# LukasHaas/PIGEON

Hardware: AMD Instinct MI355X
Metric: images/sec end-to-end (ViT+head+refine), 4x336x336 (higher is better)
Workload: dtype f16

## Files before the change

### include/pigeon_hip.h

```cpp
#ifndef PIGEON_HIP_H
#define PIGEON_HIP_H

#include <stddef.h>
#include <stdint.h>

#ifdef __cplusplus
extern "C" {
#endif

#define PG_OK            0
#define PG_EINVAL       -1
#define PG_ENOMEM       -2
#define PG_EHIP         -3
#define PG_ESTATE       -4

#define PG_DTYPE_F32     0
#define PG_DTYPE_BF16    1
#define PG_DTYPE_F16     2
#define PG_DTYPE_F64     3

#define PG_ABI_VERSION   7

const char* pg_last_error(void);
int pg_abi_version(void);
// ... 143 lines not shown
int pg_comm_rccl_version(void);

int pg_proto_build(const float* train_emb, int panels, int64_t num_train, const int64_t* member_off,
                   const int64_t* member_idx, int64_t num_protos, float* proto_emb, void* stream);
int pg_haversine_matrix(const void* x, int x_dtype, const double* y, int N, int M, double* out, void* stream);
int pg_haversine_pairs(const double* x, const void* y, int y_dtype, int64_t N, double* out, void* stream);
int pg_smooth_labels(const double* distances, int N, int M, double constant, double* out, void* stream);

int pg_haversine_blocks(const double* pts, const int64_t* cell_off, const int64_t* mat_off, int C, double zero_as, double* out,
                        void* stream);
int pg_optics_graph(const double* dist, const int64_t* cell_off, const int64_t* mat_off, int C, int min_samples, int64_t* ordering,
                    double* core, double* reach, int64_t* pred, void* stream);
int pg_optics_plan(int64_t n, int min_samples, int32_t out[4]);
int pg_tune_optics_lds_points(int max_points);

int pg_op_gemm16(int dtype, const void* A, int64_t lda, const void* W, const float* bias, void* out, int64_t ldc,
                 int M, int N, int K, int epi, float qscale, int qcols, const float* aux,
                 int variant, void* stream);
int pg_op_gemm16_ld(int dtype, const void* A, int64_t lda, const void* W, int64_t ldw, const float* bias, void* out,
                    int64_t ldc, int M, int N, int K, int epi, float qscale, int qcols, const float* aux,
                    int variant, void* stream);
int pg_op_rowstat_cast(const float* x, void* x16, int dtype, float* rowstat, int64_t rows, float eps, void* stream);
int pg_op_gemm16_resid_stat(int dtype, const void* A, int64_t lda, const void* W, int64_t ldw, const float* bias, float* X,
                            int64_t ldc, void* x16, int64_t ldx, float* statpart, int M, int N, int K, int variant, void* stream);
int pg_op_rowstat_finalize(const float* statpart, int slots, float* rowstat, int64_t rows, float eps, void* stream);
int pg_op_gemm16_ln(int dtype, const void* A, int64_t lda, const void* W, int64_t ldw, const float* bias, const float* colsum,
                    const float* rowstat, void* out, int64_t ldc, int M, int N, int K, int epi, float qscale, int qcols,
                    int variant, void* stream);
int pg_op_layernorm(const float* x, const float* gamma, const float* beta, void* y, int out_dtype,
                    int64_t rows, float eps, void* stream);
int pg_op_attention(int dtype, const void* qkv, void* out, int n_images, void* stream);
int pg_op_im2col(const void* pixels, int pix_dtype, void* out, int out_dtype, int n_images, void* stream);
int pg_op_token_mean(const float* x, float* out, int n_images, void* stream);
int pg_op_cast_f32(const float* x, void* y, int out_dtype, int64_t n, void* stream);
int pg_op_preln(float* x, const float* cls, const float* pos0, const float* gamma, const float* beta, int64_t rows, float eps,
                void* x16, int x16_dtype, float* rowstat, void* stream);
int pg_op_gemm16_parts(int dtype, const void* A, int64_t lda, const void* W, int64_t ldw, const float* bias, float* parts,
                       int M, int N, int Kp, int S, void* stream);
int pg_op_x3_split(const float* x, void* y3, int64_t rows, int cols, int gelu, void* stream);
int pg_op_x3_layernorm(const float* x, const float* gamma, const float* beta, void* y3, int64_t rows, float eps, void* stream);
int pg_op_attention_f32(const float* qkv, float* out, int n_images, void* stream);
int pg_op_attention_x3(const float* qkv, void* out3, int n_images, void* stream);
int pg_op_x3_im2col(const void* pixels, int pix_dtype, void* out3, int n_images, void* stream);
int pg_op_sum_parts(const float* parts, int S, int64_t part_elems, float* dst, int64_t n, int resid, void* stream);

#ifdef __cplusplus
}
#endif
#endif
```

### pigeon_amd/_lib.py

```python
from __future__ import annotations

import ctypes as C
import os

_HERE = os.path.dirname(os.path.abspath(__file__))
LIB_PATH = os.environ.get("PIGEON_HIP_LIB") or os.path.join(_HERE, "libpigeon_hip.so")

PG_DTYPE_F32, PG_DTYPE_BF16, PG_DTYPE_F16, PG_DTYPE_F64 = 0, 1, 2, 3
EPI_QKV, EPI_GELU, EPI_RESID, EPI_PATCH, EPI_F32, EPI_RESID_STAT, EPI_QKV_LN, EPI_GELU_LN, EPI_GELU_X3 = 0, 1, 2, 3, 4, 5, 6, 7, 8
PROF_CLASSES = ["gemm_qkv", "gemm_out", "gemm_fc1", "gemm_fc2", "gemm_patch", "attention", "layernorm",
                "im2col", "token_mean"]


class PigeonHipError(RuntimeError):
    pass


class VitCfg(C.Structure):
    _fields_ = [("layers", C.c_int32), ("image_size", C.c_int32), ("patch", C.c_int32), ("hidden", C.c_int32),
                ("heads", C.c_int32), ("mlp", C.c_int32), ("ln_eps", C.c_float), ("max_chunk", C.c_int32),
                ("mma_dtype", C.c_int32), ("precise", C.c_int32)]


class Bank(C.Structure):
# ... 64 lines not shown
    "pg_prep_ragged_destroy": (_I, [_P]),
    "pg_prep_ragged_forward": (_I, [_P, _P, _SZ, C.POINTER(PrepItem), _I, _P, _I, _P, _SZ, _P]),
    "pg_proto_build": (_I, [_P, _I, _I64, _P, _P, _I64, _P, _P]),
    "pg_haversine_matrix": (_I, [_P, _I, _P, _I, _I, _P, _P]),
    "pg_haversine_pairs": (_I, [_P, _P, _I, _I64, _P, _P]),
    "pg_smooth_labels": (_I, [_P, _I, _I, _D, _P, _P]),
    "pg_haversine_blocks": (_I, [_P, _P, _P, _I, _D, _P, _P]),
    "pg_optics_graph": (_I, [_P, _P, _P, _I, _I, _P, _P, _P, _P, _P]),
    "pg_optics_plan": (_I, [_I64, _I, C.POINTER(C.c_int32)]),
    "pg_tune_optics_lds_points": (_I, [_I]),
    "pg_head_forward": (_I, [_P, _I, _I, _P, _P, _P, _I, _I, _P, _P, _P, _P, _P, _P]),
    "pg_head_margin": (_I, [_P, _I, _I, _P, _I, _P, _P, _P, _P, _P]),
    "pg_head_certainty": (_I, [_P, _I, _I, _P, _I, _P, _P, _I, _P, _P, _P, _P, _P, _P, _P]),
    "pg_aux_heads_forward": (_I, [_P, _I, _I, _P, _P, _I, _I, _I, _P, _P, _P, _P, _P, _P, _P]),
    "pg_refine_forward": (_I, [C.POINTER(Bank), _P, _I, _I, _P, _P, _P, _I, _I, _F, _D, _P, _P, _P, _P, _P]),
    "pg_refine_forward_ex": (_I, [C.POINTER(Bank), _P, _I, _I, _P, _P, _P, _I, _I, _I, _F, _D, _P, _P, _P, _P, _P, _P]),
    "pg_refine_certainty": (_I, [C.POINTER(Bank), _P, _I, _I, _P, _P, _I, _I, _I, _P, _P, _I, _P, _P, _F, _P, _P, _P, _P, _P]),
    "pg_requeue_append": (_I, [_P, _P, _P, _I, _F, _I, _I64, _I64, _I64, _P, _P, _P, _P, _P, _P]),
    "pg_rows_to_slots": (_I, [_P, _I64, _P, _I, _P, _P]),
    "pg_requeue_take": (_I, [_P, _I64, _I64, _I, _I, _P, _P]),
    "pg_scatter_rows": (_I, [_P, _I64, _P, _I, _P, _I64, _I64, _I64, _I64, _P]),
    "pg_head_wstats": (_I, [_P, _I, _P, _P, _P]),
    "pg_embedding_debias": (_I, [_P, _I64, _I, _P, _P]),
    "pg_op_gemm16": (_I, [_I, _P, _I64, _P, _P, _P, _I64, _I, _I, _I, _I, _F, _I, _P, _I, _P]),
    "pg_op_gemm16_ld": (_I, [_I, _P, _I64, _P, _I64, _P, _P, _I64, _I, _I, _I, _I, _F, _I, _P, _I, _P]),
    "pg_op_rowstat_cast": (_I, [_P, _P, _I, _P, _I64, _F, _P]),
    "pg_op_gemm16_resid_stat": (_I, [_I, _P, _I64, _P, _I64, _P, _P, _I64, _P, _I64, _P, _I, _I, _I, _I, _P]),
    "pg_op_rowstat_finalize": (_I, [_P, _I, _P, _I64, _F, _P]),
    "pg_op_gemm16_ln": (_I, [_I, _P, _I64, _P, _I64, _P, _P, _P, _P, _I64, _I, _I, _I, _I, _F, _I, _I, _P]),
    "pg_op_layernorm": (_I, [_P, _P, _P, _P, _I, _I64, _F, _P]),
    "pg_op_attention": (_I, [_I, _P, _P, _I, _P]),
    "pg_op_im2col": (_I, [_P, _I, _P, _I, _I, _P]),
    "pg_op_token_mean": (_I, [_P, _P, _I, _P]),
    "pg_op_cast_f32": (_I, [_P, _P, _I, _I64, _P]),
    "pg_op_gemm16_parts": (_I, [_I, _P, _I64, _P, _I64, _P, _P, _I, _I, _I, _I, _P]),
    "pg_op_x3_split": (_I, [_P, _P, _I64, _I, _I, _P]),
    "pg_op_x3_layernorm": (_I, [_P, _P, _P, _P, _I64, _F, _P]),
    "pg_op_attention_f32": (_I, [_P, _P, _I, _P]),
    "pg_op_attention_x3": (_I, [_P, _P, _I, _P]),
    "pg_op_x3_im2col": (_I, [_P, _I, _P, _I, _P]),
    "pg_op_sum_parts": (_I, [_P, _I, _I64, _P, _I64, _I, _P]),
    "pg_op_preln": (_I, [_P, _P, _P, _P, _P, _I64, _F, _P, _I, _P, _P]),
    "pg_vit_precise_plan": (_I, [_I, C.POINTER(C.c_int32)]),
}

_lib = None


def load():
    global _lib
    if _lib is not None:
        return _lib
    if not os.path.exists(LIB_PATH):
        raise PigeonHipError(
            f"{LIB_PATH} not found: build it with `python -m pigeon_amd.build` (hipcc, gfx950). "
            "pigeon_amd has no CPU/PyTorch fallback for its hot path.")
    import torch
    lib = C.CDLL(LIB_PATH)
    for name, (res, args) in SIGNATURES.items():
        fn = getattr(lib, name)
        fn.restype = res
        fn.argtypes = args
    _lib = lib
    return lib


# ... 14 lines not shown
```

### pigeon_amd/build.py

```python
from __future__ import annotations

import os
import subprocess
import sys
from concurrent.futures import ThreadPoolExecutor

HERE = os.path.dirname(os.path.abspath(__file__))
CSRC = os.path.join(HERE, "csrc")
OBJ = os.path.join(CSRC, "build")
LIB = os.path.join(HERE, "libpigeon_hip.so")
SOURCES = ["vit.hip", "gemm_plan.hip", "gemm_bf16.hip", "gemm_pp.hip", "gemm_pp6.hip", "gemm_tail.hip", "gemm_mid.hip", "attention.hip", "rowops.hip", "precise.hip",
           "preprocess.hip", "geo_proto.hip", "head.hip", "refine.hip", "certainty.hip", "aux_heads.hip", "requeue.hip", "fingerprint.hip", "comm.hip", "optics.hip"]
HEADERS = [os.path.join(CSRC, "common.h"), os.path.join(CSRC, "pigeon_internal.h"), os.path.join(CSRC, "gemm_epi.h"),
           os.path.join(CSRC, "attention_common.h"), os.path.join(CSRC, "certainty_common.h"),
           os.path.join(os.path.dirname(HERE), "include", "pigeon_hip.h")]
FLAGS = ["--offload-arch=gfx950", "-O3", "-std=c++17", "-fPIC", "-Wall", "-Wno-unused-function"]


def hipcc() -> str:
    for c in (os.environ.get("HIPCC"), "/opt/rocm/bin/hipcc", "hipcc"):
        if c and (os.path.isabs(c) and os.path.exists(c) or not os.path.isabs(c)):
            return c
    return "hipcc"


def _stale(target: str, deps) -> bool:
    if not os.path.exists(target):
        return True
    t = os.path.getmtime(target)
    return any(os.path.getmtime(d) > t for d in deps)


def build(force: bool = False, verbose: bool = True, dev: bool = False) -> str:
    global OBJ, LIB
    obj_dir = os.path.join(CSRC, "build_dev" if dev else "build")
    lib = os.path.join(HERE, "libpigeon_hip_dev.so" if dev else "libpigeon_hip.so")
    flags = FLAGS + (["-DPIGEON_PROBES"] if dev else [])
    return _build(obj_dir, lib, flags, force, verbose, SOURCES)


def _build(OBJ: str, LIB: str, FLAGS, force: bool, verbose: bool, SOURCES) -> str:
    os.makedirs(OBJ, exist_ok=True)
    cc = hipcc()
    jobs = []
# ... 43 lines not shown
```

### pigeon_amd/csrc/pigeon_internal.h

```cpp
#pragma once
#include <hip/hip_runtime.h>
#include <stdint.h>
#include "../../include/pigeon_hip.h"

enum { EPI_QKV = 0, EPI_GELU = 1, EPI_RESID = 2, EPI_PATCH = 3, EPI_F32 = 4, EPI_RESID_STAT = 5, EPI_QKV_LN = 6, EPI_GELU_LN = 7,
       EPI_GELU_X3 = 8 };

struct PgGemmExtra {
    const float* colsum = nullptr;
    const float* rowstat = nullptr;
    void* x16 = nullptr;
    int64_t ldx = 0;
    float* statpart = nullptr;
    int64_t stat_rows = 0;
    int parts = 1;
    int64_t a_part = 0, w_part = 0, c_part = 0;
};

void pg_set_error(const char* fmt, ...) __attribute__((format(printf, 1, 2)));
int pg_check_launch(const char* what);
int pg_default_gemm_variant();
int pg_gemm_grid_cus();
int pg_gemm_raster_gn();
unsigned long long pg_tune_epoch();
int pg_gemm_precise_route(int M, int N, int Ktot, bool resid, const int* cand, int ncand);

enum { PG_GEMM_V_ONE_TILE = 8, PG_GEMM_V_PP = 36, PG_GEMM_V_PP6 = 56, PG_GEMM_V_TAIL = 70, PG_GEMM_V_MID = 71 };
enum PgGemmKernel { PG_GK_NONE = -1, PG_GK_PP6 = 0, PG_GK_PP = 1, PG_GK_MID = 2, PG_GK_TAIL = 3, PG_GK_ONE_TILE = 4 };

#define PG_HIP(call)                                                                          \
    do {                                                                                      \
        hipError_t e__ = (call);                                                              \
        if (e__ != hipSuccess) {                                                              \
            pg_set_error("%s failed: %s (%s:%d)", #call, hipGetErrorString(e__), __FILE__, __LINE__); \
            return PG_EHIP;                                                                   \
        }                                                                                     \
    } while (0)

struct PgFpBuf { const void* data; size_t bytes; uint64_t seed; };
int pg_fingerprint_many(const PgFpBuf* bufs, int n, uint64_t* out, hipStream_t stream);
void pg_fingerprint_host(const void* data, size_t bytes, uint64_t seed, uint64_t out[2]);

int pg_gemm_launch(int dtype, const void* A, int64_t lda, const void* W, int64_t ldw, const float* bias, void* out, int64_t ldc,
                   int M, int N, int K, int epi, float qscale, int qcols, const float* aux, int variant,
                   hipStream_t s, const PgGemmExtra* extra = nullptr);
int pg_layernorm_launch(const float* x, const float* gamma, const float* beta, void* y, int out_dtype,
                        int64_t rows, float eps, hipStream_t s);
int pg_preln_launch(float* x, const float* cls, const float* pos0, const float* gamma, const float* beta,
                    int64_t rows, float eps, hipStream_t s, void* x16 = nullptr, int x16_dtype = 0, float* rowstat = nullptr);
int pg_im2col_launch(const void* pixels, int pix_dtype, void* out, int out_dtype, int n_images, hipStream_t s);
int pg_token_mean_launch(const float* x, float* out, int n_images, hipStream_t s);
int pg_cast_f32_launch(const float* x, void* y, int out_dtype, int64_t n, hipStream_t s);
int pg_rowstat_cast_launch(const float* x, void* x16, int out_dtype, float* rowstat, int64_t rows, float eps, hipStream_t s);
int pg_rowstat_finalize_launch(const float* statpart, int slots, float* rowstat, int64_t rows, float eps, hipStream_t s,
                               unsigned long long* alarm = nullptr, float alarm_sumsq = 0.f);
int pg_count_sat16_launch(const void* buf, int64_t rows, int cols, int64_t ld, int dtype, unsigned long long* counter, hipStream_t s);
int pg_attention_launch(int dtype, const void* qkv, void* out, int n_images, hipStream_t s);
int pg_x3_ln_launch(const float* x, const float* gamma, const float* beta, void* y3, int64_t rows, float eps, hipStream_t s);
int pg_x3_split_launch(const float* x, void* y3, int64_t rows, int C, int gelu, hipStream_t s);
int pg_x3_im2col_launch(const void* pixels, int pix_dtype, void* out3, int n_images, hipStream_t s);
int pg_attention_f32_launch(const float* qkv, float* out, int n_images, hipStream_t s);
bool pg_attention_x3out_available();
int pg_attention_x3out_launch(const float* qkv, void* out3, int n_images, hipStream_t s);
int pg_sum_parts_launch(const float* parts, int S, int64_t part_elems, float* dst, int64_t n, int resid, hipStream_t s);
```

### pigeon_amd/csrc/rowops.hip

```cpp
#include "common.h"
#include "pigeon_internal.h"

template <int OUT>
__global__ __launch_bounds__(256) void layernorm_kernel(const float* __restrict__ x, const float* __restrict__ gamma,
                                                        const float* __restrict__ beta, void* __restrict__ y,
                                                        int64_t rows, float eps) {
    const int lane = threadIdx.x & 63;
    const int64_t row = (int64_t)blockIdx.x * 4 + (threadIdx.x >> 6);
    if (row >= rows) return;
    const float* xr = x + row * VIT_HIDDEN;
    f32x4 v[4];
#pragma unroll
    for (int i = 0; i < 4; ++i) v[i] = *(const f32x4*)(xr + i * 256 + lane * 4);
    float s = 0.f;
#pragma unroll
    for (int i = 0; i < 4; ++i) s += (v[i][0] + v[i][1]) + (v[i][2] + v[i][3]);
    const float mean = wave_sum(s) * (1.0f / VIT_HIDDEN);
    float q = 0.f;
#pragma unroll
    for (int i = 0; i < 4; ++i)
#pragma unroll
        for (int e = 0; e < 4; ++e) { const float d = v[i][e] - mean; q += d * d; }
    const float var = wave_sum(q) * (1.0f / VIT_HIDDEN);
    const float rstd = 1.0f / sqrtf(var + eps);
// ... 200 lines not shown
    } else { pg_set_error("im2col: unsupported pixel dtype %d", pix_dtype); return PG_EINVAL; }
    return pg_check_launch("im2col");
}

__global__ __launch_bounds__(256) void token_mean_kernel(const float* __restrict__ x, float* __restrict__ out) {
    const int img = blockIdx.x >> 2, col = (blockIdx.x & 3) * 256 + threadIdx.x;
    const float* p = x + (int64_t)img * VIT_TOKENS * VIT_HIDDEN + col;
    float s0 = 0.f, s1 = 0.f, s2 = 0.f, s3 = 0.f;
    int t = 0;
    for (; t + 16 <= VIT_TOKENS; t += 16) {
        float v[16];
#pragma unroll
        for (int i = 0; i < 16; ++i) v[i] = p[(int64_t)(t + i) * VIT_HIDDEN];
#pragma unroll
        for (int i = 0; i < 16; i += 4) { s0 += v[i]; s1 += v[i + 1]; s2 += v[i + 2]; s3 += v[i + 3]; }
    }
    for (; t + 4 <= VIT_TOKENS; t += 4) {
        s0 += p[(int64_t)(t + 0) * VIT_HIDDEN];
        s1 += p[(int64_t)(t + 1) * VIT_HIDDEN];
        s2 += p[(int64_t)(t + 2) * VIT_HIDDEN];
        s3 += p[(int64_t)(t + 3) * VIT_HIDDEN];
    }
    for (; t < VIT_TOKENS; ++t) s0 += p[(int64_t)t * VIT_HIDDEN];
    out[(int64_t)img * VIT_HIDDEN + col] = ((s0 + s1) + (s2 + s3)) / (float)VIT_TOKENS;
}

int pg_token_mean_launch(const float* x, float* out, int n_images, hipStream_t s) {
    if (n_images <= 0) return PG_OK;
    hipLaunchKernelGGL(token_mean_kernel, dim3(n_images * 4), dim3(256), 0, s, x, out);
    return pg_check_launch("token_mean");
}

template <typename T>
__global__ __launch_bounds__(256) void f32_to_16_kernel(const float* __restrict__ x, uint16_t* __restrict__ y, int64_t n) {
    int64_t i = ((int64_t)blockIdx.x * 256 + threadIdx.x) * 4;
    const int64_t stride = (int64_t)gridDim.x * 256 * 4;
    for (; i + 3 < n; i += stride) {
        const f32x4 v = *(const f32x4*)(x + i);
        u32x2 pk;
        pk[0] = pack16x2<T>(v[0], v[1]);
        pk[1] = pack16x2<T>(v[2], v[3]);
        *(u32x2*)(y + i) = pk;
    }
    if (i < n) for (int64_t j = i; j < n; ++j) y[j] = T::bits(x[j]);
}

int pg_cast_f32_launch(const float* x, void* y, int out_dtype, int64_t n, hipStream_t s) {
    if (n <= 0) return PG_OK;
    int64_t blocks = (n / 4 + 255) / 256;
    if (blocks > 4096) blocks = 4096;
    if (blocks < 1) blocks = 1;
    if (out_dtype == PG_DTYPE_F16) hipLaunchKernelGGL(f32_to_16_kernel<T_F16>, dim3((unsigned)blocks), dim3(256), 0, s, x, (uint16_t*)y, n);
    else if (out_dtype == PG_DTYPE_BF16) hipLaunchKernelGGL(f32_to_16_kernel<T_BF16>, dim3((unsigned)blocks), dim3(256), 0, s, x, (uint16_t*)y, n);
    else { pg_set_error("cast: bad output dtype %d", out_dtype); return PG_EINVAL; }
    return pg_check_launch("cast_f32");
}

__global__ __launch_bounds__(256) void count_sat16_kernel(const uint16_t* __restrict__ buf, int64_t rows, int cols, int64_t ld,
                                                          int is_f16, unsigned long long* __restrict__ counter) {
    const int64_t vec_per_row = cols / 8;
    const int64_t total = rows * vec_per_row;
    unsigned long long n = 0;
    for (int64_t i = (int64_t)blockIdx.x * 256 + threadIdx.x; i < total; i += (int64_t)gridDim.x * 256) {
        const int64_t r = i / vec_per_row, c = (i - r * vec_per_row) * 8;
        const u32x4 v = *(const u32x4*)(buf + r * ld + c);
#pragma unroll
// ... 19 lines not shown
```

### pigeon_amd/csrc/vit.hip

```cpp
#include "common.h"
#include "pigeon_internal.h"

#include <cmath>
#include <cstdarg>
#include <cstdio>
#include <cstdlib>
#include <cstring>
#include <map>
#include <string>
#include <vector>

static thread_local char g_err[512] = "";

void pg_set_error(const char* fmt, ...) {
    va_list ap;
    va_start(ap, fmt);
    vsnprintf(g_err, sizeof(g_err), fmt, ap);
    va_end(ap);
}
int pg_check_launch(const char* what) {
    hipError_t e = hipGetLastError();
    if (e != hipSuccess) { pg_set_error("launch of %s failed: %s", what, hipGetErrorString(e)); return PG_EHIP; }
    return PG_OK;
}
// ... 344 lines not shown
      RC(pg_gemm_launch(dt, big, VIT_PATCH_KPAD, h->wpatch, VIT_PATCH_KPAD, nullptr, X, VIT_HIDDEN, n * VIT_PATCHES, VIT_HIDDEN, VIT_PATCH_KPAD,
                        EPI_PATCH, 1.f, 0, h->pos, 0, s)); }
    if (!h->ln_fold) { ProfScope p(h, s, 6); RC(pg_preln_launch(X, h->cls, h->pos, h->preg, h->preb, M, eps, s)); }
    if (h->ln_fold) {
        uint16_t* Xn2 = (uint16_t*)((char*)big + align_up((size_t)M * VIT_MLP * 2, 256));
        float* statpart = (float*)((char*)Xn2 + align_up((size_t)M * VIT_HIDDEN * 2, 256));
        float* rsA = (float*)((char*)statpart + align_up((size_t)M * (VIT_HIDDEN / 64) * 8, 256));
        float* rsB = (float*)((char*)rsA + align_up((size_t)M * 8, 256));
        const int slots = VIT_HIDDEN / 64;
        { ProfScope p(h, s, 6); RC(pg_preln_launch(X, h->cls, h->pos, h->preg, h->preb, M, eps, s, Xn, dt, rsA)); }
        SAT(Xn, M, VIT_HIDDEN, VIT_HIDDEN);
        for (int l = 0; l < h->cfg.layers; ++l) {
            const LayerW& L = h->layers[l];
            const bool last = l + 1 == h->cfg.layers;
            PgGemmExtra ex;
            { ProfScope p(h, s, 0);
              ex = PgGemmExtra(); ex.colsum = L.sqkv; ex.rowstat = rsA;
              RC(pg_gemm_launch(dt, Xn, VIT_HIDDEN, L.wqkv, VIT_HIDDEN, L.bqkv, big, 3 * VIT_HIDDEN, (int)M, 3 * VIT_HIDDEN, VIT_HIDDEN,
                                EPI_QKV_LN, kQScale, VIT_HIDDEN, nullptr, 0, s, &ex)); }
            SAT(big, M, 3 * VIT_HIDDEN, 3 * VIT_HIDDEN);
            { ProfScope p(h, s, 5); RC(pg_attention_launch(dt, big, Xn, n, s)); }
            SAT(Xn, M, VIT_HIDDEN, VIT_HIDDEN);
            { ProfScope p(h, s, 1);
              ex = PgGemmExtra(); ex.x16 = Xn2; ex.ldx = VIT_HIDDEN; ex.statpart = statpart;
              RC(pg_gemm_launch(dt, Xn, VIT_HIDDEN, L.wo, VIT_HIDDEN, L.bo, X, VIT_HIDDEN, (int)M, VIT_HIDDEN, VIT_HIDDEN, EPI_RESID_STAT,
                                1.f, 0, nullptr, 0, s, &ex)); }
            SAT(Xn2, M, VIT_HIDDEN, VIT_HIDDEN);
            { ProfScope p(h, s, 6); RC(pg_rowstat_finalize_launch(statpart, slots, rsB, M, eps, s, h->range_alarm, h->range_alarm_sumsq)); }
            { ProfScope p(h, s, 2);
              ex = PgGemmExtra(); ex.colsum = L.s1; ex.rowstat = rsB;
              RC(pg_gemm_launch(dt, Xn2, VIT_HIDDEN, L.w1, VIT_HIDDEN, L.b1, big, VIT_MLP, (int)M, VIT_MLP, VIT_HIDDEN, EPI_GELU_LN, 1.f, 0,
                                nullptr, 0, s, &ex)); }
            SAT(big, M, VIT_MLP, VIT_MLP);
            { ProfScope p(h, s, 3);
              if (last) {
                  RC(pg_gemm_launch(dt, big, VIT_MLP, L.w2, VIT_MLP, L.b2, X, VIT_HIDDEN, (int)M, VIT_HIDDEN, VIT_MLP, EPI_RESID, 1.f, 0, nullptr, 0, s));
              } else {
                  ex = PgGemmExtra(); ex.x16 = Xn; ex.ldx = VIT_HIDDEN; ex.statpart = statpart;
                  RC(pg_gemm_launch(dt, big, VIT_MLP, L.w2, VIT_MLP, L.b2, X, VIT_HIDDEN, (int)M, VIT_HIDDEN, VIT_MLP, EPI_RESID_STAT, 1.f, 0,
                                    nullptr, 0, s, &ex));
              } }
            if (!last) SAT(Xn, M, VIT_HIDDEN, VIT_HIDDEN);
            if (!last) { ProfScope p(h, s, 6); RC(pg_rowstat_finalize_launch(statpart, slots, rsA, M, eps, s, h->range_alarm, h->range_alarm_sumsq)); }
        }
    } else
    for (int l = 0; l < h->cfg.layers; ++l) {
        const LayerW& L = h->layers[l];
        { ProfScope p(h, s, 6); RC(pg_layernorm_launch(X, L.ln1g, L.ln1b, Xn, dt, M, eps, s)); }
        SAT(Xn, M, VIT_HIDDEN, VIT_HIDDEN);
        { ProfScope p(h, s, 0);
          RC(pg_gemm_launch(dt, Xn, VIT_HIDDEN, L.wqkv, VIT_HIDDEN, L.bqkv, big, 3 * VIT_HIDDEN, (int)M, 3 * VIT_HIDDEN, VIT_HIDDEN, EPI_QKV,
                            kQScale, VIT_HIDDEN, nullptr, 0, s)); }
        SAT(big, M, 3 * VIT_HIDDEN, 3 * VIT_HIDDEN);
        { ProfScope p(h, s, 5); RC(pg_attention_launch(dt, big, Xn, n, s)); }
        SAT(Xn, M, VIT_HIDDEN, VIT_HIDDEN);
        { ProfScope p(h, s, 1);
          RC(pg_gemm_launch(dt, Xn, VIT_HIDDEN, L.wo, VIT_HIDDEN, L.bo, X, VIT_HIDDEN, (int)M, VIT_HIDDEN, VIT_HIDDEN, EPI_RESID, 1.f, 0, nullptr, 0, s)); }
        { ProfScope p(h, s, 6); RC(pg_layernorm_launch(X, L.ln2g, L.ln2b, Xn, dt, M, eps, s)); }
        SAT(Xn, M, VIT_HIDDEN, VIT_HIDDEN);
        { ProfScope p(h, s, 2);
          RC(pg_gemm_launch(dt, Xn, VIT_HIDDEN, L.w1, VIT_HIDDEN, L.b1, big, VIT_MLP, (int)M, VIT_MLP, VIT_HIDDEN, EPI_GELU, 1.f, 0, nullptr, 0, s)); }
        SAT(big, M, VIT_MLP, VIT_MLP);
        { ProfScope p(h, s, 3);
          RC(pg_gemm_launch(dt, big, VIT_MLP, L.w2, VIT_MLP, L.b2, X, VIT_HIDDEN, (int)M, VIT_HIDDEN, VIT_MLP, EPI_RESID, 1.f, 0, nullptr, 0, s)); }
    }
    return PG_OK;
}

static void graph_entry_free(pg_vit::GraphEntry& e) {
    if (e.done) { (void)hipEventSynchronize(e.done); (void)hipEventDestroy(e.done); }
    if (e.exec) (void)hipGraphExecDestroy(e.exec);
    if (e.graph) (void)hipGraphDestroy(e.graph);
    e.exec = nullptr; e.graph = nullptr; e.done = nullptr;
}
static int vit_forward_body_graphed(pg_vit* h, int n, char* ws, hipStream_t s) {
    const bool ok = h->use_graph && !h->prof && !h->sat_check && h->streams == 1;
    if (!ok) return vit_forward_body(h, n, ws, s);
    pg_vit::GraphEntry* ent = nullptr;
    for (auto& e : h->graphs) if (e.ws == ws && e.n == n) { ent = &e; break; }
    if (!ent) {
        if (h->graphs.size() >= 8) {
            size_t lru = 0;
            for (size_t i = 1; i < h->graphs.size(); ++i) if (h->graphs[i].last_use < h->graphs[lru].last_use) lru = i;
            graph_entry_free(h->graphs[lru]);
            h->graphs.erase(h->graphs.begin() + lru);
        }
        h->graphs.push_back({ws, n, 0, nullptr, nullptr, 0, pg_tune_epoch(), nullptr});
        ent = &h->graphs.back();
    }
    ent->last_use = ++h->graph_clock;
    if (ent->exec && ent->epoch != pg_tune_epoch()) {
        graph_entry_free(*ent);
        ent->seen = 1;
    }
    if (ent->exec) {
// ... 5 lines not shown
    if (ent->seen++ == 0) return vit_forward_body(h, n, ws, s);
    if (!h->capture_stream) PG_HIP(hipStreamCreateWithFlags(&h->capture_stream, hipStreamNonBlocking));
    hipGraph_t graph = nullptr;
    hipError_t e = hipStreamBeginCapture(h->capture_stream, hipStreamCaptureModeThreadLocal);
    if (e != hipSuccess) { (void)hipGetLastError(); h->use_graph = false; return vit_forward_body(h, n, ws, s); }
    const int rc = vit_forward_body(h, n, ws, h->capture_stream);
    e = hipStreamEndCapture(h->capture_stream, &graph);
    if (rc != PG_OK || e != hipSuccess || !graph) {
        (void)hipGetLastError();
        if (graph) (void)hipGraphDestroy(graph);
        h->use_graph = false;
        return vit_forward_body(h, n, ws, s);
    }
    hipGraphExec_t exec = nullptr;
    e = hipGraphInstantiate(&exec, graph, nullptr, nullptr, 0);
    if (e != hipSuccess || !exec) { (void)hipGetLastError(); (void)hipGraphDestroy(graph); h->use_graph = false; return vit_forward_body(h, n, ws, s); }
    ent->graph = graph; ent->exec = exec; ent->epoch = pg_tune_epoch();
    if (!ent->done) (void)hipEventCreateWithFlags(&ent->done, hipEventDisableTiming);
    ++h->graph_captures;
    PG_HIP(hipGraphLaunch(exec, s));
    if (ent->done) (void)hipEventRecord(ent->done, s);
    ++h->graph_replays;
    return PG_OK;
}

static int vit_forward_chunk(pg_vit* h, const void* pixels, int pix_dtype, int n, float* emb_out, float* hidden_out,
                             char* ws, hipStream_t s) {
    const int64_t M = (int64_t)n * VIT_TOKENS;
    float* X = (float*)ws;
    uint16_t* Xn = (uint16_t*)(ws + align_up((size_t)M * VIT_HIDDEN * 4, 256));
    uint16_t* big = (uint16_t*)((char*)Xn + align_up((size_t)M * VIT_HIDDEN * 2, 256));
    { ProfScope p(h, s, 7); RC(pg_im2col_launch(pixels, pix_dtype, big, h->cfg.mma_dtype, n, s)); }
    RC(vit_forward_body_graphed(h, n, ws, s));
    { ProfScope p(h, s, 8); RC(pg_token_mean_launch(X, emb_out, n, s)); }
    if (hidden_out) PG_HIP(hipMemcpyAsync(hidden_out, X, (size_t)M * VIT_HIDDEN * 4, hipMemcpyDeviceToDevice, s));
    return PG_OK;
}

extern "C" int pg_vit_forward_hidden(pg_vit* h, const void* pixels, int pix_dtype, int n_images, float* emb_out,
                                     float* hidden_out, void* workspace, size_t workspace_bytes, void* stream) {
    if (!h) { pg_set_error("vit_forward: null handle"); return PG_EINVAL; }
    if (!h->finalized) { pg_set_error("vit_forward: handle not finalized"); return PG_ESTATE; }
    if (n_images < 0) { pg_set_error("vit_forward: n_images = %d", n_images); return PG_EINVAL; }
    if (n_images == 0) return PG_OK;
    if (!pixels || !emb_out || !workspace) { pg_set_error("vit_forward: null argument"); return PG_EINVAL; }
    if (pix_dtype != PG_DTYPE_F32 && pix_dtype != PG_DTYPE_BF16 && pix_dtype != PG_DTYPE_F16) { pg_set_error("vit_forward: bad pixel dtype"); return PG_EINVAL; }
    size_t needb = 0;
    pg_vit_workspace_bytes(h, n_images, &needb);
    if (workspace_bytes < needb) { pg_set_error("vit_forward: workspace %zu < required %zu bytes", workspace_bytes, needb); return PG_ENOMEM; }
    if (((uintptr_t)workspace & 255) != 0) { pg_set_error("vit_forward: workspace must be 256-byte aligned"); return PG_EINVAL; }
    hipStream_t s = (hipStream_t)stream;
    const size_t esz = pix_dtype == PG_DTYPE_F32 ? 4 : 2;
    const size_t img_elems = (size_t)3 * VIT_IMG * VIT_IMG;
    auto run_range = [&](int first, int last, char* ws, hipStream_t st) -> int {
        for (int s0 = first; s0 < last; s0 += h->cfg.max_chunk) {
            const int n = (last - s0) < h->cfg.max_chunk ? (last - s0) : h->cfg.max_chunk;
            RC(vit_forward_chunk(h, (const char*)pixels + (size_t)s0 * img_elems * esz, pix_dtype, n,
                                 emb_out + (size_t)s0 * VIT_HIDDEN,
                                 hidden_out ? hidden_out + (size_t)s0 * VIT_TOKENS * VIT_HIDDEN : nullptr, ws, st));
        }
        return PG_OK;
    };
    const int parts = split_parts(h, n_images);
    if (parts > 1) {
        const int per = (n_images + parts - 1) / parts;
        const size_t wsp = needb / parts;
        PG_HIP(hipEventRecord(h->ev_fork, s));
        for (int i = 0; i + 1 < parts; ++i) PG_HIP(hipStreamWaitEvent(h->sx[i], h->ev_fork, 0));
// ... 319 lines not shown
                                       int64_t ldc, void* x16, int64_t ldx, float* statpart, int M, int N, int K, int variant,
                                       void* stream) {
    if (!A || !W || !X || !x16 || !statpart) { pg_set_error("op_gemm16_resid_stat: null argument"); return PG_EINVAL; }
    PgGemmExtra ex; ex.x16 = x16; ex.ldx = ldx; ex.statpart = statpart;
    return pg_gemm_launch(dtype, A, lda, W, ldw, bias, X, ldc, M, N, K, EPI_RESID_STAT, 1.f, 0, nullptr, variant ? variant : PG_GEMM_V_PP,
                          (hipStream_t)stream, &ex);
}
extern "C" int pg_op_gemm16_ln(int dtype, const void* A, int64_t lda, const void* W, int64_t ldw, const float* bias,
                               const float* colsum, const float* rowstat, void* out, int64_t ldc, int M, int N, int K, int epi,
                               float qscale, int qcols, int variant, void* stream) {
    if (!A || !W || !out || !colsum || !rowstat) { pg_set_error("op_gemm16_ln: null argument"); return PG_EINVAL; }
    if (epi != EPI_QKV_LN && epi != EPI_GELU_LN) { pg_set_error("op_gemm16_ln: epi must be 6 or 7"); return PG_EINVAL; }
    PgGemmExtra ex; ex.colsum = colsum; ex.rowstat = rowstat;
    return pg_gemm_launch(dtype, A, lda, W, ldw, bias, out, ldc, M, N, K, epi, qscale, qcols, nullptr, variant ? variant : PG_GEMM_V_PP,
                          (hipStream_t)stream, &ex);
}
extern "C" int pg_op_layernorm(const float* x, const float* gamma, const float* beta, void* y, int out_dtype,
                               int64_t rows, float eps, void* stream) {
    if (!x || !gamma || !beta || !y) { pg_set_error("op_layernorm: null argument"); return PG_EINVAL; }
    return pg_layernorm_launch(x, gamma, beta, y, out_dtype, rows, eps, (hipStream_t)stream);
}
extern "C" int pg_op_attention(int dtype, const void* qkv, void* out, int n_images, void* stream) {
    if (!qkv || !out) { pg_set_error("op_attention: null argument"); return PG_EINVAL; }
    return pg_attention_launch(dtype, qkv, out, n_images, (hipStream_t)stream);
}
extern "C" int pg_op_im2col(const void* pixels, int pix_dtype, void* out, int out_dtype, int n_images, void* stream) {
    if (!pixels || !out) { pg_set_error("op_im2col: null argument"); return PG_EINVAL; }
    return pg_im2col_launch(pixels, pix_dtype, out, out_dtype, n_images, (hipStream_t)stream);
}
extern "C" int pg_op_token_mean(const float* x, float* out, int n_images, void* stream) {
    if (!x || !out) { pg_set_error("op_token_mean: null argument"); return PG_EINVAL; }
    return pg_token_mean_launch(x, out, n_images, (hipStream_t)stream);
}
extern "C" int pg_op_cast_f32(const float* x, void* y, int out_dtype, int64_t n, void* stream) {
    if (!x || !y) { pg_set_error("op_cast_f32: null argument"); return PG_EINVAL; }
    return pg_cast_f32_launch(x, y, out_dtype, n, (hipStream_t)stream);
}

extern "C" int pg_op_gemm16_parts(int dtype, const void* A, int64_t lda, const void* W, int64_t ldw, const float* bias, float* parts,
                                  int M, int N, int Kp, int S, void* stream) {
    if (!A || !W || !parts) { pg_set_error("op_gemm16_parts: null argument"); return PG_EINVAL; }
    if (S < 1 || S > 8) { pg_set_error("op_gemm16_parts: 1 <= S <= 8"); return PG_EINVAL; }
    PgGemmExtra ex;
    ex.parts = S; ex.a_part = Kp; ex.w_part = Kp; ex.c_part = (int64_t)M * N;
    return pg_gemm_launch(dtype, A, lda, W, ldw, bias, parts, N, M, N, Kp, EPI_F32, 1.f, 0, nullptr, PG_GEMM_V_PP, (hipStream_t)stream, &ex);
}

extern "C" int pg_op_x3_split(const float* x, void* y3, int64_t rows, int cols, int gelu, void* stream) {
    if (!x || !y3) { pg_set_error("op_x3_split: null argument"); return PG_EINVAL; }
    return pg_x3_split_launch(x, y3, rows, cols, gelu, (hipStream_t)stream);
}
extern "C" int pg_op_x3_layernorm(const float* x, const float* gamma, const float* beta, void* y3, int64_t rows, float eps, void* stream) {
    if (!x || !gamma || !beta || !y3) { pg_set_error("op_x3_layernorm: null argument"); return PG_EINVAL; }
    return pg_x3_ln_launch(x, gamma, beta, y3, rows, eps, (hipStream_t)stream);
}
extern "C" int pg_op_attention_f32(const float* qkv, float* out, int n_images, void* stream) {
    if (!qkv || !out) { pg_set_error("op_attention_f32: null argument"); return PG_EINVAL; }
    return pg_attention_f32_launch(qkv, out, n_images, (hipStream_t)stream);
}
extern "C" int pg_op_x3_im2col(const void* pixels, int pix_dtype, void* out3, int n_images, void* stream) {
    if (!pixels || !out3 || n_images < 0) { pg_set_error("op_x3_im2col: bad argument"); return PG_EINVAL; }
    return pg_x3_im2col_launch(pixels, pix_dtype, out3, n_images, (hipStream_t)stream);
}
extern "C" int pg_op_sum_parts(const float* parts, int S, int64_t part_elems, float* dst, int64_t n, int resid, void* stream) {
    if (!parts || !dst) { pg_set_error("op_sum_parts: null argument"); return PG_EINVAL; }
    if (S < 1 || S > 8 || n < 0 || n > part_elems) { pg_set_error("op_sum_parts: 1 <= S <= 8, 0 <= n <= part_elems"); return PG_EINVAL; }
// ... 13 lines not shown
```

### pigeon_amd/hip_ops.py

```python
from __future__ import annotations

import ctypes as C
from typing import Dict, Optional

import torch

from . import _lib
from ._lib import Bank, VitCfg, check, load

TOKENS, HIDDEN, MLP, PATCHES, KPAD = 577, 1024, 4096, 576, 640


def _p(t: Optional[torch.Tensor]):
    return C.c_void_p(0) if t is None else C.c_void_p(t.data_ptr())


def _stream():
    return C.c_void_p(torch.cuda.current_stream().cuda_stream)


_T16 = {torch.float16: _lib.PG_DTYPE_F16, torch.bfloat16: _lib.PG_DTYPE_BF16}
_PIXDT = {torch.float32: _lib.PG_DTYPE_F32, torch.float16: _lib.PG_DTYPE_F16, torch.bfloat16: _lib.PG_DTYPE_BF16}
_PG2T = {_lib.PG_DTYPE_F16: torch.float16, _lib.PG_DTYPE_BF16: torch.bfloat16, _lib.PG_DTYPE_F32: torch.float32}

# ... 98 lines not shown

def layernorm(x: torch.Tensor, gamma: torch.Tensor, beta: torch.Tensor, eps: float = 1e-5,
              out_dtype: torch.dtype = torch.float16, out: Optional[torch.Tensor] = None) -> torch.Tensor:
    _dev(x, torch.float32)
    rows = x.numel() // HIDDEN
    if out is None:
        out = torch.empty(x.shape, dtype=out_dtype, device=x.device)
    pg = _lib.PG_DTYPE_F32 if out.dtype == torch.float32 else _dt16(out)
    check(load().pg_op_layernorm(_p(x), _p(gamma), _p(beta), _p(out), pg, rows, float(eps), _stream()), "pg_op_layernorm")
    return out


def attention(qkv: torch.Tensor, n_images: int) -> torch.Tensor:
    _dev(qkv)
    out = torch.empty((n_images * TOKENS, HIDDEN), dtype=qkv.dtype, device=qkv.device)
    check(load().pg_op_attention(_dt16(qkv), _p(qkv), _p(out), n_images, _stream()), "pg_op_attention")
    return out


def im2col(pixels: torch.Tensor, out_dtype: torch.dtype = torch.float16) -> torch.Tensor:
    _dev(pixels)
    n = pixels.shape[0]
    dt = _PIXDT[pixels.dtype]
    out = torch.empty((n * PATCHES, KPAD), dtype=out_dtype, device=pixels.device)
    check(load().pg_op_im2col(_p(pixels), dt, _p(out), _dt16(out), n, _stream()), "pg_op_im2col")
    return out


def token_mean(x: torch.Tensor) -> torch.Tensor:
    _dev(x, torch.float32)
    n = x.shape[0]
    out = torch.empty((n, HIDDEN), dtype=torch.float32, device=x.device)
    check(load().pg_op_token_mean(_p(x), _p(out), n, _stream()), "pg_op_token_mean")
    return out


def cast_f32(x: torch.Tensor, out_dtype: torch.dtype = torch.float16) -> torch.Tensor:
    _dev(x, torch.float32)
    y = torch.empty(x.shape, dtype=out_dtype, device=x.device)
    check(load().pg_op_cast_f32(_p(x), _p(y), _dt16(y), x.numel(), _stream()), "pg_op_cast_f32")
    return y


def proto_build(train_emb: torch.Tensor, member_off: torch.Tensor, member_idx: torch.Tensor) -> torch.Tensor:
    _dev(train_emb, torch.float32); _dev(member_off, torch.int64); _dev(member_idx, torch.int64)
    if train_emb.dim() not in (2, 3) or train_emb.shape[-1] != HIDDEN:
        raise _lib.PigeonHipError(f"proto_build: embeddings must be (Ntr,{HIDDEN}) or (Ntr,panels,{HIDDEN}), got {tuple(train_emb.shape)}")
    panels = 1 if train_emb.dim() == 2 else int(train_emb.shape[1])
    if member_off.dim() != 1 or member_off.numel() < 1 or member_idx.dim() != 1:
        raise _lib.PigeonHipError("proto_build: member_off (P+1,) and member_idx (n,) expected")
    P = member_off.numel() - 1
    off = member_off.cpu()
    if int(off[0]) != 0 or int(off[-1]) != member_idx.numel() or bool((off[1:] < off[:-1]).any()):
        raise _lib.PigeonHipError("proto_build: member_off must rise from 0 to len(member_idx)")
    if member_idx.numel() and (int(member_idx.min()) < 0 or int(member_idx.max()) >= train_emb.shape[0]):
        raise _lib.PigeonHipError(f"proto_build: member index outside the {train_emb.shape[0]} training rows")
    out = torch.empty((P, HIDDEN), dtype=torch.float32, device=train_emb.device)
    check(load().pg_proto_build(_p(train_emb), panels, train_emb.shape[0], _p(member_off), _p(member_idx), P, _p(out),
                                _stream()), "pg_proto_build")
    return out


def haversine_matrix(x: torch.Tensor, y_rows: torch.Tensor) -> torch.Tensor:
    _dev(x); _dev(y_rows, torch.float64)
    if x.dtype not in (torch.float32, torch.float64):
        raise _lib.PigeonHipError("haversine_matrix: x must be fp32 or fp64")
# ... 729 lines not shown
```

Measured before the change: 2498.

## Replace last-layer fc2 GEMM with token-mean then small GEMV via linearity

The final block's fc2 GEMM plus residual is linear, so its token mean equals fc2 applied to the mean of the GELU activations, plus the mean residual and bias. The last-layer fc2 GEMM over all tokens is skipped. Instead, the code averages X and the f16 MLP activations across tokens and runs a small fused GEMV kernel to produce the embedding. This removes a full M x 4096 x 1024 GEMM per forward. The full GEMM still runs when hidden states are requested, and summation order differs from the reference path.

```diff
diff --git a/include/pigeon_hip.h b/include/pigeon_hip.h
--- a/include/pigeon_hip.h
+++ b/include/pigeon_hip.h
@@ -199,6 +199,9 @@
 int pg_op_attention(int dtype, const void* qkv, void* out, int n_images, void* stream);
 int pg_op_im2col(const void* pixels, int pix_dtype, void* out, int out_dtype, int n_images, void* stream);
 int pg_op_token_mean(const float* x, float* out, int n_images, void* stream);
+int pg_op_token_mean16(const void* x16, int dtype, int cols, float* out, int n_images, void* stream);
+int pg_op_mean_tail(const float* xbar, const float* hbar, const void* w2, int dtype, const float* b2, float* out, int n, int K, int N,
+                    void* stream);
 int pg_op_cast_f32(const float* x, void* y, int out_dtype, int64_t n, void* stream);
 int pg_op_preln(float* x, const float* cls, const float* pos0, const float* gamma, const float* beta, int64_t rows, float eps,
                 void* x16, int x16_dtype, float* rowstat, void* stream);
diff --git a/pigeon_amd/_lib.py b/pigeon_amd/_lib.py
--- a/pigeon_amd/_lib.py
+++ b/pigeon_amd/_lib.py
@@ -120,6 +120,8 @@
     "pg_op_attention": (_I, [_I, _P, _P, _I, _P]),
     "pg_op_im2col": (_I, [_P, _I, _P, _I, _I, _P]),
     "pg_op_token_mean": (_I, [_P, _P, _I, _P]),
+    "pg_op_token_mean16": (_I, [_P, _I, _I, _P, _I, _P]),
+    "pg_op_mean_tail": (_I, [_P, _P, _P, _I, _P, _P, _I, _I, _I, _P]),
     "pg_op_cast_f32": (_I, [_P, _P, _I, _I64, _P]),
     "pg_op_gemm16_parts": (_I, [_I, _P, _I64, _P, _I64, _P, _P, _I, _I, _I, _I, _P]),
     "pg_op_x3_split": (_I, [_P, _P, _I64, _I, _I, _P]),
diff --git a/pigeon_amd/build.py b/pigeon_amd/build.py
--- a/pigeon_amd/build.py
+++ b/pigeon_amd/build.py
@@ -9,7 +9,7 @@
 CSRC = os.path.join(HERE, "csrc")
 OBJ = os.path.join(CSRC, "build")
 LIB = os.path.join(HERE, "libpigeon_hip.so")
-SOURCES = ["vit.hip", "gemm_plan.hip", "gemm_bf16.hip", "gemm_pp.hip", "gemm_pp6.hip", "gemm_tail.hip", "gemm_mid.hip", "attention.hip", "rowops.hip", "precise.hip",
+SOURCES = ["vit.hip", "gemm_plan.hip", "gemm_bf16.hip", "gemm_pp.hip", "gemm_pp6.hip", "gemm_tail.hip", "gemm_mid.hip", "attention.hip", "rowops.hip", "mean_tail.hip", "precise.hip",
            "preprocess.hip", "geo_proto.hip", "head.hip", "refine.hip", "certainty.hip", "aux_heads.hip", "requeue.hip", "fingerprint.hip", "comm.hip", "optics.hip"]
 HEADERS = [os.path.join(CSRC, "common.h"), os.path.join(CSRC, "pigeon_internal.h"), os.path.join(CSRC, "gemm_epi.h"),
            os.path.join(CSRC, "attention_common.h"), os.path.join(CSRC, "certainty_common.h"),
diff --git a/pigeon_amd/csrc/mean_tail.hip b/pigeon_amd/csrc/mean_tail.hip
--- /dev/null
+++ b/pigeon_amd/csrc/mean_tail.hip
@@ -0,0 +1,91 @@
+#include "common.h"
+#include "pigeon_internal.h"
+
+template <typename T, int CN>
+__global__ __launch_bounds__(64) void mean_tail_kernel(const float* __restrict__ xbar, const float* __restrict__ hbar,
+                                                       const uint16_t* __restrict__ w2, const float* __restrict__ b2,
+                                                       float* __restrict__ out, int n, int K, int N) {
+    const int lane = threadIdx.x;
+    const int c0 = blockIdx.x * CN, i0 = blockIdx.y * 8;
+    const int ni = (n - i0) < 8 ? (n - i0) : 8;
+    float acc[8][CN];
+#pragma unroll
+    for (int i = 0; i < 8; ++i)
+#pragma unroll
+        for (int c = 0; c < CN; ++c) acc[i][c] = 0.f;
+    const uint16_t* wp = w2 + (int64_t)c0 * K;
+    const float* hp = hbar + (int64_t)i0 * K;
+#pragma unroll 2
+    for (int k = lane * 8; k < K; k += 64 * 8) {
+        float w[CN][8];
+#pragma unroll
+        for (int c = 0; c < CN; ++c) {
+            const u32x4 v = *(const u32x4*)(wp + (int64_t)c * K + k);
+#pragma unroll
+            for (int e = 0; e < 4; ++e) {
+                w[c][2 * e] = T::val((uint16_t)(v[e] & 0xffffu));
+                w[c][2 * e + 1] = T::val((uint16_t)(v[e] >> 16));
+            }
+        }
+#pragma unroll
+        for (int i = 0; i < 8; ++i) {
+            if (i < ni) {
+                const f32x4 h0 = *(const f32x4*)(hp + (int64_t)i * K + k);
+                const f32x4 h1 = *(const f32x4*)(hp + (int64_t)i * K + k + 4);
+#pragma unroll
+                for (int c = 0; c < CN; ++c) {
+#pragma unroll
+                    for (int e = 0; e < 4; ++e) acc[i][c] = __builtin_fmaf(h0[e], w[c][e], acc[i][c]);
+#pragma unroll
+                    for (int e = 0; e < 4; ++e) acc[i][c] = __builtin_fmaf(h1[e], w[c][4 + e], acc[i][c]);
+                }
+            }
+        }
+    }
+    float mine[CN];
+#pragma unroll
+    for (int c = 0; c < CN; ++c) mine[c] = 0.f;
+#pragma unroll
+    for (int i = 0; i < 8; ++i) {
+        if (i < ni) {
+#pragma unroll
+            for (int c = 0; c < CN; ++c) {
+                const float v = wave_sum(acc[i][c]);
+                if (lane == i) mine[c] = v;
+            }
+        }
+    }
+    if (lane < ni) {
+        const int64_t o = (int64_t)(i0 + lane) * N + c0;
+#pragma unroll
+        for (int c = 0; c < CN; c += 4) {
+            const f32x4 b = *(const f32x4*)(b2 + c0 + c);
+            const f32x4 x = *(const f32x4*)(xbar + o + c);
+            f32x4 r;
+#pragma unroll
+            for (int e = 0; e < 4; ++e) r[e] = (mine[c + e] + b[e]) + x[e];
+            *(f32x4*)(out + o + c) = r;
+        }
+    }
+}
+
+int pg_mean_tail_launch(const float* xbar, const float* hbar, const void* w2, int dtype, const float* b2, float* out, int n, int K,
+                        int N, hipStream_t s) {
+    if (n <= 0) return PG_OK;
+    if (K <= 0 || (K & 7) != 0 || N <= 0 || (N & 7) != 0) { pg_set_error("mean_tail: K = %d, N = %d must be positive multiples of 8", K, N); return PG_EINVAL; }
+    if (dtype != PG_DTYPE_F16 && dtype != PG_DTYPE_BF16) { pg_set_error("mean_tail: bad dtype %d", dtype); return PG_EINVAL; }
+    const int tiles = (n + 7) / 8;
+    if (tiles > 65535) { pg_set_error("mean_tail: n = %d exceeds %d", n, 8 * 65535); return PG_EINVAL; }
+    const bool h = dtype == PG_DTYPE_F16;
+    const uint16_t* w = (const uint16_t*)w2;
+    if (n <= 8) {
+        const dim3 grid(N / 4, tiles);
+        if (h) hipLaunchKernelGGL((mean_tail_kernel<T_F16, 4>), grid, dim3(64), 0, s, xbar, hbar, w, b2, out, n, K, N);
+        else hipLaunchKernelGGL((mean_tail_kernel<T_BF16, 4>), grid, dim3(64), 0, s, xbar, hbar, w, b2, out, n, K, N);
+    } else {
+        const dim3 grid(N / 8, tiles);
+        if (h) hipLaunchKernelGGL((mean_tail_kernel<T_F16, 8>), grid, dim3(64), 0, s, xbar, hbar, w, b2, out, n, K, N);
+        else hipLaunchKernelGGL((mean_tail_kernel<T_BF16, 8>), grid, dim3(64), 0, s, xbar, hbar, w, b2, out, n, K, N);
+    }
+    return pg_check_launch("mean_tail");
+}
diff --git a/pigeon_amd/csrc/pigeon_internal.h b/pigeon_amd/csrc/pigeon_internal.h
--- a/pigeon_amd/csrc/pigeon_internal.h
+++ b/pigeon_amd/csrc/pigeon_internal.h
@@ -50,6 +50,9 @@
                     int64_t rows, float eps, hipStream_t s, void* x16 = nullptr, int x16_dtype = 0, float* rowstat = nullptr);
 int pg_im2col_launch(const void* pixels, int pix_dtype, void* out, int out_dtype, int n_images, hipStream_t s);
 int pg_token_mean_launch(const float* x, float* out, int n_images, hipStream_t s);
+int pg_token_mean16_launch(const void* x16, int dtype, int cols, float* out, int n_images, hipStream_t s);
+int pg_mean_tail_launch(const float* xbar, const float* hbar, const void* w2, int dtype, const float* b2, float* out, int n, int K,
+                        int N, hipStream_t s);
 int pg_cast_f32_launch(const float* x, void* y, int out_dtype, int64_t n, hipStream_t s);
 int pg_rowstat_cast_launch(const float* x, void* x16, int out_dtype, float* rowstat, int64_t rows, float eps, hipStream_t s);
 int pg_rowstat_finalize_launch(const float* statpart, int slots, float* rowstat, int64_t rows, float eps, hipStream_t s,
diff --git a/pigeon_amd/csrc/rowops.hip b/pigeon_amd/csrc/rowops.hip
--- a/pigeon_amd/csrc/rowops.hip
+++ b/pigeon_amd/csrc/rowops.hip
@@ -256,6 +256,58 @@
 }
 
 template <typename T>
+__device__ __forceinline__ void add16x8(float (&a)[8], const u32x4 v) {
+#pragma unroll
+    for (int e = 0; e < 4; ++e) {
+        a[2 * e] += T::val((uint16_t)(v[e] & 0xffffu));
+        a[2 * e + 1] += T::val((uint16_t)(v[e] >> 16));
+    }
+}
+
+template <typename T>
+__global__ __launch_bounds__(256) void token_mean16_kernel(const uint16_t* __restrict__ x, float* __restrict__ out, int cols) {
+    __shared__ float part[32][64];
+    const int img = blockIdx.y, c0 = blockIdx.x * 64;
+    const int j = threadIdx.x & 7, g = threadIdx.x >> 3;
+    const int c = c0 + j * 8;
+    const bool live = c < cols;
+    float a[8] = {0.f, 0.f, 0.f, 0.f, 0.f, 0.f, 0.f, 0.f};
+    if (live) {
+        const uint16_t* p = x + ((int64_t)img * VIT_TOKENS + g) * cols + c;
+        u32x4 v[18];
+#pragma unroll
+        for (int i = 0; i < 18; ++i) v[i] = *(const u32x4*)(p + (int64_t)i * 32 * cols);
+#pragma unroll
+        for (int i = 0; i < 18; ++i) add16x8<T>(a, v[i]);
+        if (g == 0) add16x8<T>(a, *(const u32x4*)(p + (int64_t)576 * cols));
+    }
+    *(f32x4*)&part[g][j * 8] = f32x4{a[0], a[1], a[2], a[3]};
+    *(f32x4*)&part[g][j * 8 + 4] = f32x4{a[4], a[5], a[6], a[7]};
+    __syncthreads();
+    if (threadIdx.x < 64 && c0 + (int)threadIdx.x < cols) {
+        float q[32];
+#pragma unroll
+        for (int k = 0; k < 32; ++k) q[k] = part[k][threadIdx.x];
+#pragma unroll
+        for (int s = 16; s >= 1; s >>= 1)
+#pragma unroll
+            for (int k = 0; k < s; ++k) q[k] += q[k + s];
+        out[(int64_t)img * cols + c0 + threadIdx.x] = q[0] / (float)VIT_TOKENS;
+    }
+}
+
+int pg_token_mean16_launch(const void* x16, int dtype, int cols, float* out, int n_images, hipStream_t s) {
+    if (n_images <= 0) return PG_OK;
+    if (cols <= 0 || (cols & 7) != 0) { pg_set_error("token_mean16: cols = %d is not a positive multiple of 8", cols); return PG_EINVAL; }
+    if (n_images > 65535) { pg_set_error("token_mean16: n_images = %d exceeds 65535", n_images); return PG_EINVAL; }
+    const dim3 grid((cols + 63) / 64, n_images);
+    if (dtype == PG_DTYPE_F16) hipLaunchKernelGGL(token_mean16_kernel<T_F16>, grid, dim3(256), 0, s, (const uint16_t*)x16, out, cols);
+    else if (dtype == PG_DTYPE_BF16) hipLaunchKernelGGL(token_mean16_kernel<T_BF16>, grid, dim3(256), 0, s, (const uint16_t*)x16, out, cols);
+    else { pg_set_error("token_mean16: bad dtype %d", dtype); return PG_EINVAL; }
+    return pg_check_launch("token_mean16");
+}
+
+template <typename T>
 __global__ __launch_bounds__(256) void f32_to_16_kernel(const float* __restrict__ x, uint16_t* __restrict__ y, int64_t n) {
     int64_t i = ((int64_t)blockIdx.x * 256 + threadIdx.x) * 4;
     const int64_t stride = (int64_t)gridDim.x * 256 * 4;
diff --git a/pigeon_amd/csrc/vit.hip b/pigeon_amd/csrc/vit.hip
--- a/pigeon_amd/csrc/vit.hip
+++ b/pigeon_amd/csrc/vit.hip
@@ -400,16 +400,13 @@
               RC(pg_gemm_launch(dt, Xn2, VIT_HIDDEN, L.w1, VIT_HIDDEN, L.b1, big, VIT_MLP, (int)M, VIT_MLP, VIT_HIDDEN, EPI_GELU_LN, 1.f, 0,
                                 nullptr, 0, s, &ex)); }
             SAT(big, M, VIT_MLP, VIT_MLP);
+            if (last) break;
             { ProfScope p(h, s, 3);
-              if (last) {
-                  RC(pg_gemm_launch(dt, big, VIT_MLP, L.w2, VIT_MLP, L.b2, X, VIT_HIDDEN, (int)M, VIT_HIDDEN, VIT_MLP, EPI_RESID, 1.f, 0, nullptr, 0, s));
-              } else {
-                  ex = PgGemmExtra(); ex.x16 = Xn; ex.ldx = VIT_HIDDEN; ex.statpart = statpart;
-                  RC(pg_gemm_launch(dt, big, VIT_MLP, L.w2, VIT_MLP, L.b2, X, VIT_HIDDEN, (int)M, VIT_HIDDEN, VIT_MLP, EPI_RESID_STAT, 1.f, 0,
-                                    nullptr, 0, s, &ex));
-              } }
-            if (!last) SAT(Xn, M, VIT_HIDDEN, VIT_HIDDEN);
-            if (!last) { ProfScope p(h, s, 6); RC(pg_rowstat_finalize_launch(statpart, slots, rsA, M, eps, s, h->range_alarm, h->range_alarm_sumsq)); }
+              ex = PgGemmExtra(); ex.x16 = Xn; ex.ldx = VIT_HIDDEN; ex.statpart = statpart;
+              RC(pg_gemm_launch(dt, big, VIT_MLP, L.w2, VIT_MLP, L.b2, X, VIT_HIDDEN, (int)M, VIT_HIDDEN, VIT_MLP, EPI_RESID_STAT, 1.f, 0,
+                                nullptr, 0, s, &ex)); }
+            SAT(Xn, M, VIT_HIDDEN, VIT_HIDDEN);
+            { ProfScope p(h, s, 6); RC(pg_rowstat_finalize_launch(statpart, slots, rsA, M, eps, s, h->range_alarm, h->range_alarm_sumsq)); }
         }
     } else
     for (int l = 0; l < h->cfg.layers; ++l) {
@@ -429,6 +426,7 @@
         { ProfScope p(h, s, 2);
           RC(pg_gemm_launch(dt, Xn, VIT_HIDDEN, L.w1, VIT_HIDDEN, L.b1, big, VIT_MLP, (int)M, VIT_MLP, VIT_HIDDEN, EPI_GELU, 1.f, 0, nullptr, 0, s)); }
         SAT(big, M, VIT_MLP, VIT_MLP);
+        if (l + 1 == h->cfg.layers) break;
         { ProfScope p(h, s, 3);
           RC(pg_gemm_launch(dt, big, VIT_MLP, L.w2, VIT_MLP, L.b2, X, VIT_HIDDEN, (int)M, VIT_HIDDEN, VIT_MLP, EPI_RESID, 1.f, 0, nullptr, 0, s)); }
     }
@@ -500,8 +498,19 @@
     uint16_t* big = (uint16_t*)((char*)Xn + align_up((size_t)M * VIT_HIDDEN * 2, 256));
     { ProfScope p(h, s, 7); RC(pg_im2col_launch(pixels, pix_dtype, big, h->cfg.mma_dtype, n, s)); }
     RC(vit_forward_body_graphed(h, n, ws, s));
-    { ProfScope p(h, s, 8); RC(pg_token_mean_launch(X, emb_out, n, s)); }
-    if (hidden_out) PG_HIP(hipMemcpyAsync(hidden_out, X, (size_t)M * VIT_HIDDEN * 4, hipMemcpyDeviceToDevice, s));
+    const LayerW& L = h->layers[h->cfg.layers - 1];
+    float* xbar = (float*)Xn;
+    float* hbar = xbar + (size_t)n * VIT_HIDDEN;
+    { ProfScope p(h, s, 8);
+      RC(pg_token_mean_launch(X, xbar, n, s));
+      RC(pg_token_mean16_launch(big, h->cfg.mma_dtype, VIT_MLP, hbar, n, s));
+      RC(pg_mean_tail_launch(xbar, hbar, L.w2, h->cfg.mma_dtype, L.b2, emb_out, n, VIT_MLP, VIT_HIDDEN, s)); }
+    if (hidden_out) {
+        { ProfScope p(h, s, 3);
+          RC(pg_gemm_launch(h->cfg.mma_dtype, big, VIT_MLP, L.w2, VIT_MLP, L.b2, X, VIT_HIDDEN, (int)M, VIT_HIDDEN, VIT_MLP, EPI_RESID, 1.f, 0,
+                            nullptr, 0, s)); }
+        PG_HIP(hipMemcpyAsync(hidden_out, X, (size_t)M * VIT_HIDDEN * 4, hipMemcpyDeviceToDevice, s));
+    }
     return PG_OK;
 }
 
@@ -887,6 +896,19 @@
     if (!x || !out) { pg_set_error("op_token_mean: null argument"); return PG_EINVAL; }
     return pg_token_mean_launch(x, out, n_images, (hipStream_t)stream);
 }
+extern "C" int pg_op_token_mean16(const void* x16, int dtype, int cols, float* out, int n_images, void* stream) {
+    if (!x16 || !out) { pg_set_error("op_token_mean16: null argument"); return PG_EINVAL; }
+    if (((uintptr_t)x16 & 15) != 0 || ((uintptr_t)out & 15) != 0) { pg_set_error("op_token_mean16: buffers must be 16-byte aligned"); return PG_EINVAL; }
+    return pg_token_mean16_launch(x16, dtype, cols, out, n_images, (hipStream_t)stream);
+}
+extern "C" int pg_op_mean_tail(const float* xbar, const float* hbar, const void* w2, int dtype, const float* b2, float* out, int n, int K,
+                               int N, void* stream) {
+    if (!xbar || !hbar || !w2 || !b2 || !out) { pg_set_error("op_mean_tail: null argument"); return PG_EINVAL; }
+    if ((((uintptr_t)xbar | (uintptr_t)hbar | (uintptr_t)w2 | (uintptr_t)b2 | (uintptr_t)out) & 15) != 0) {
+        pg_set_error("op_mean_tail: buffers must be 16-byte aligned"); return PG_EINVAL;
+    }
+    return pg_mean_tail_launch(xbar, hbar, w2, dtype, b2, out, n, K, N, (hipStream_t)stream);
+}
 extern "C" int pg_op_cast_f32(const float* x, void* y, int out_dtype, int64_t n, void* stream) {
     if (!x || !y) { pg_set_error("op_cast_f32: null argument"); return PG_EINVAL; }
     return pg_cast_f32_launch(x, y, out_dtype, n, (hipStream_t)stream);
diff --git a/pigeon_amd/hip_ops.py b/pigeon_amd/hip_ops.py
--- a/pigeon_amd/hip_ops.py
+++ b/pigeon_amd/hip_ops.py
@@ -154,6 +154,31 @@
     n = x.shape[0]
     out = torch.empty((n, HIDDEN), dtype=torch.float32, device=x.device)
     check(load().pg_op_token_mean(_p(x), _p(out), n, _stream()), "pg_op_token_mean")
+    return out
+
+
+def token_mean16(x: torch.Tensor) -> torch.Tensor:
+    _dev(x)
+    _shape(x, "token_mean16: x", None, TOKENS, None)
+    n, cols = int(x.shape[0]), int(x.shape[2])
+    if cols <= 0 or cols % 8:
+        raise _lib.PigeonHipError(f"token_mean16: cols = {cols} must be a positive multiple of 8")
+    out = torch.empty((n, cols), dtype=torch.float32, device=x.device)
+    check(load().pg_op_token_mean16(_p(x), _dt16(x), cols, _p(out), n, _stream()), "pg_op_token_mean16")
+    return out
+
+
+def mean_tail(xbar: torch.Tensor, hbar: torch.Tensor, w2: torch.Tensor, b2: torch.Tensor) -> torch.Tensor:
+    _dev(xbar, torch.float32); _dev(hbar, torch.float32); _dev(w2); _dev(b2, torch.float32)
+    if w2.dim() != 2:
+        raise _lib.PigeonHipError(f"mean_tail: w2 must be (N,K), got {tuple(w2.shape)}")
+    N, K = int(w2.shape[0]), int(w2.shape[1])
+    if K <= 0 or K % 8 or N <= 0 or N % 8:
+        raise _lib.PigeonHipError(f"mean_tail: K = {K} and N = {N} must be positive multiples of 8")
+    n = int(xbar.shape[0])
+    _shape(xbar, "mean_tail: xbar", n, N); _shape(hbar, "mean_tail: hbar", n, K); _shape(b2, "mean_tail: b2", N)
+    out = torch.empty((n, N), dtype=torch.float32, device=xbar.device)
+    check(load().pg_op_mean_tail(_p(xbar), _p(hbar), _p(w2), _dt16(w2), _p(b2), _p(out), n, K, N, _stream()), "pg_op_mean_tail")
     return out
 
 
```

Result: no change. 2516 (median of 6 runs) (+0.7%).
